# gabegrand/VQA-Counterexamples

Measured on AMD Instinct MI355X. Metric: VQA-CX triplets/sec (24 candidates each), NeuralCX training step, higher is better.
Workload: dtype f32; 1 GPU; configs[1]: NeuralCX MLP train step (fwd+listwise loss/recall+bwd+Adam), synthetic 2048-d feats, 24 candidates, batch 512 per GPU (weak scaling: global batch 512), H=256, L=1, dropout 0.25, fp32; global_batch=512, per_rank_batch=512, candidates=24, dim_h=256, n_layers=1, parallelism=dp1, feature_table_rows=82783

## Files before the change

### vqa-counterexamples_amd/csrc/ncx_api.hip

```cpp
#include "ncx_internal.h"
#include "ncx_dwred.h"
#include "ncx_bf16.h"
#include <stdlib.h>
#include <stdio.h>
#include <atomic>

namespace ncx {

template <int CTRL> __device__ __forceinline__ float dpp_mov(float v) {
    return __builtin_bit_cast(float, __builtin_amdgcn_update_dpp(0, __builtin_bit_cast(int, v), CTRL, 0xF, 0xF, false));
}
__device__ __forceinline__ float lane_bcast(float v, int lane) {
    return __builtin_bit_cast(float, __builtin_amdgcn_readlane(__builtin_bit_cast(int, v), lane));
}
__device__ __forceinline__ float wave_sum(float v) {
    v += dpp_mov<0xB1>(v); v += dpp_mov<0x4E>(v); v += dpp_mov<0x141>(v); v += dpp_mov<0x140>(v);
    return (lane_bcast(v, 0) + lane_bcast(v, 16)) + (lane_bcast(v, 32) + lane_bcast(v, 48));
}
__device__ __forceinline__ float wave_max(float v) {
    v = fmaxf(v, dpp_mov<0xB1>(v)); v = fmaxf(v, dpp_mov<0x4E>(v)); v = fmaxf(v, dpp_mov<0x141>(v)); v = fmaxf(v, dpp_mov<0x140>(v));
    return fmaxf(fmaxf(lane_bcast(v, 0), lane_bcast(v, 16)), fmaxf(lane_bcast(v, 32), lane_bcast(v, 48)));
}

__device__ __forceinline__ u16 f32_to_bf16(float x) { return __builtin_bit_cast(u16, (__bf16)x); }
// ... 542 lines not shown
    if (__syncthreads_or(earlier)) return;
    const int nw = (B + 31) / 32;
    for (int w = threadIdx.x; w < nw; w += 256) bits[w] = 0u;
    __syncthreads();
    for (int j = b + threadIdx.x; j < B; j += 256)
        if (aid[j] == id) atomicOr(&bits[j >> 5], 1u << (j & 31));
    __syncthreads();
    for (int n = threadIdx.x; n < H; n += 256) {
        float s = 0.f;
        for (int w = b >> 5; w < nw; ++w) {
            unsigned m = bits[w];
            while (m) {
                const int j = (w << 5) + __ffs(m) - 1;
                m &= m - 1;
                s += dsh[(long long)j * H + n];
            }
        }
        dggt[(long long)n * A + id] = s;
    }
}

struct EmbPrepArgs {
    const float* dsh; const int* aid; float* dggtT;
    const float* src[3]; float* dst[3]; long long lds_[3]; int cols[3], ldd[3], dcols[3], tile0[4];
    int B, H, A, Hp4;
};
__global__ __launch_bounds__(256) void k_emb_prep(const EmbPrepArgs a, const FixupArgs fix, const Tn8ReduceArgs red) {
    __shared__ unsigned bits[NCX_SCATTER_MAX_B / 32 > 32 * 33 ? NCX_SCATTER_MAX_B / 32 : 32 * 33];
    if ((int)blockIdx.x >= a.B + a.tile0[3]) {
        const int id = blockIdx.x - (a.B + a.tile0[3]);
        const int nfix = fix.valid ? fix.grid_x * 4 : 0;
        if (id < nfix) split_fixup_body<64, 64>(fix, id / 4, id % 4);
        else tn8_reduce_body(red, id - nfix);
        return;
    }
    if ((int)blockIdx.x < a.B) {
        const int b = blockIdx.x, B = a.B;
        const int id = a.aid[b];
        int earlier = 0;
        for (int j = threadIdx.x; j < b; j += 256) earlier |= a.aid[j] == id;
        if (__syncthreads_or(earlier)) return;
        const int nw = (B + 31) / 32;
        for (int w = threadIdx.x; w < nw; w += 256) bits[w] = 0u;
        __syncthreads();
        for (int j = b + threadIdx.x; j < B; j += 256)
            if (a.aid[j] == id) atomicOr(&bits[j >> 5], 1u << (j & 31));
        __syncthreads();
        for (int n = threadIdx.x; n < a.H; n += 256) {
            float s = 0.f;
            for (int w = b >> 5; w < nw; ++w) {
                unsigned m = bits[w];
                while (m) { const int j = (w << 5) + __ffs(m) - 1; m &= m - 1; s += a.dsh[(long long)j * a.H + n]; }
            }
            a.dggtT[(long long)id * a.Hp4 + n] = s;
        }
        return;
    }
    float* tile = (float*)bits;
    int t = blockIdx.x - a.B, e = 0;
    while (e < 2 && t >= a.tile0[e + 1]) ++e;
    t -= a.tile0[e];
    const int tiles_h = (a.dcols[e] + 31) / 32;
    const int th = t % tiles_h, tc = t / tiles_h;
    const int x = threadIdx.x & 31, y = threadIdx.x >> 5;
#pragma unroll
    for (int i = 0; i < 4; ++i) {
        const int h = th * 32 + y + 8 * i, c = tc * 32 + x;
        tile[(y + 8 * i) * 33 + x] = (h < a.H && c < a.cols[e]) ? a.src[e][(long long)h * a.lds_[e] + c] : 0.f;
    }
    __syncthreads();
#pragma unroll
    for (int i = 0; i < 4; ++i) {
        const int c = tc * 32 + y + 8 * i, h = th * 32 + x;
        if (c < a.cols[e] && h < a.dcols[e]) a.dst[e][(long long)c * a.ldd[e] + h] = tile[x * 33 + y + 8 * i];
    }
}

__global__ __launch_bounds__(256) void k_zero_cols(float* __restrict__ p, int rows, long long ld, int cols) {
    const long long i = (long long)blockIdx.x * 256 + threadIdx.x;
    if (i >= (long long)rows * cols) return;
    const int r = (int)(i / cols), c = (int)(i - (long long)r * cols);
    p[(long long)r * ld + c] = 0.f;
}

__global__ __launch_bounds__(256) void k_adam(float* __restrict__ p, const float* __restrict__ g, float* __restrict__ m,
                                              float* __restrict__ v, size_t n, float step_size, float b1, float b2,
                                              float eps, float inv_bc2_sqrt, float gscale) {
    size_t i = ((size_t)blockIdx.x * 256 + threadIdx.x) * 4;
    const size_t stride = (size_t)gridDim.x * 256 * 4;
    for (; i < n; i += stride) {
        if (i + 3 < n) {
            f32x4 pv = *(f32x4*)(p + i), gv = *(const f32x4*)(g + i), mv = *(f32x4*)(m + i), vv = *(f32x4*)(v + i);
#pragma unroll
            for (int j = 0; j < 4; ++j) {
                const float gj = gv[j] * gscale;
                mv[j] = mv[j] + (gj - mv[j]) * (1.f - b1);
                vv[j] = vv[j] * b2 + (1.f - b2) * gj * gj;
                const float den = sqrtf(vv[j]) * inv_bc2_sqrt + eps;
// ... 154 lines not shown
        } else {
            wgs = WgMap{(int)cdiv(u[i].M, bm), (int)cdiv(u[i].N, bn), S}.count();
        }
        u[i].wgs = wgs;
        u[i].slab_elems = S > 1 ? wgs * bm * bn : 0;
    }
    u[U_DW1S].plan.cfg = u[U_DW1C].plan.cfg;
    {
        int bm, bn; cfg_tile(u[U_DW1C].plan.cfg, bm, bn);
        const bool tn8 = dw_tn8_shared_ok(d);
        const long long segs_s[4] = {tn8 ? 0 : d.dv, tn8 ? 0 : d.dq, tn8 ? 0 : d.dz, tn8 ? 0 : d.da};
        const int S = u[U_DW1S].plan.split > 1 ? u[U_DW1S].plan.split : 1;
        u[U_DW1S].tiles = 0; u[U_DW1S].wgs = 0;
        for (int q = 0; q < 4; ++q) {
            if (segs_s[q] == 0) continue;
            u[U_DW1S].tiles += cdiv(H, bm) * cdiv(segs_s[q], bn);
            u[U_DW1S].wgs += WgMap{(int)cdiv(H, bm), (int)cdiv(segs_s[q], bn), S}.count();
        }
        u[U_DW1C].slab_elems = (u[U_DW1C].wgs + u[U_DW1S].wgs) * bm * bn;
        u[U_DW1S].slab_elems = 0;
    }
}

WsLayout ws_layout(const ncx_dims& d) {
    WsLayout w{};
    const size_t M = (size_t)d.B * d.K, H = d.H;
    size_t off = 0;
    auto take = [&](size_t bytes) { size_t o = off; off = align_up(off + bytes, 256); return o; };
    w.idx_k = take(M * 4); w.idx_o = take(M * 4); w.idx_ob = take((size_t)d.B * 4);
    w.mx = take(M * 4); w.inv = take(M * 4);
    w.ldm = pad_to(d.K + 1, 4);
    w.ldgt = (d.flags & NCX_F_BF16) ? d.A : pad_to(d.A, 32);
    w.misc = take(M * w.ldm * 4);
    w.gt = take(H * w.ldgt * 4);
    w.sh = take((size_t)d.B * H * 4);
    for (int l = 0; l < 3; ++l) w.h[l] = l < d.L ? take(M * H * 4) : 0;
    w.dpre[0] = take(M * H * 4);
    w.dpre[1] = d.L >= 2 ? take(M * H * 4) : 0;
    w.dsh = take((size_t)d.B * H * 4);
    w.dgt = take(2 * H * d.A * 4);
    w.dagt = w.dgt + H * d.A * 4;
    w.dgtT = take((size_t)2 * d.A * pad_to(d.H, 4) * 4);
    w.w1aT = take((size_t)2 * d.da * pad_to(d.H, 32) * 4);
    w.dgtT2 = take(dw_tn8_supported(d) ? (size_t)pad_to(d.A, 32) * pad_to(d.H, 4) * 4 : 0);
    w.partial = take((size_t)NCX_PRELUDE_WAVES * H * 4 * 2 + (size_t)NCX_PRELUDE_WAVES * 4 + 256);
    GemmUse u[U_COUNT];
    list_uses(d, u);
    long long slab = 0;
    for (int i = 0; i < U_COUNT; ++i) slab = u[i].slab_elems > slab ? u[i].slab_elems : slab;
    w.slab_bytes = (size_t)slab * 4;
    if (dw_tn8_slab_bytes(d) > w.slab_bytes) w.slab_bytes = dw_tn8_slab_bytes(d);
    w.slab = take(w.slab_bytes);
    {
        long long s2 = u[U_GT].slab_elems;
        if (u[U_SH].slab_elems > s2) s2 = u[U_SH].slab_elems;
        if (u[U_DW1AK].slab_elems > s2) s2 = u[U_DW1AK].slab_elems;
        if (u[U_DE].slab_elems > s2) s2 = u[U_DE].slab_elems;
        w.slab2_bytes = (size_t)s2 * 4;
        w.slab2 = take(w.slab2_bytes);
    }
    w.km_slab = take(dw_km_slab_bytes(d));
    {
        const long long Tm = ks(d.dv) * ((d.flags & NCX_F_V_MULT) ? 2 : 1) + ks(pad_to(d.K + 1, 4)) + ks(d.dz) + ((d.flags & NCX_F_A_EMB) ? ks(d.A) : ks(d.da));
        auto need = [&](long long m, long long n, long long t) { const int sp = main_split(m, n, t); return sp > 1 ? (size_t)sp * m * n * 4 : (size_t)0; };
        size_t b = need((long long)M, (long long)H, Tm);
// ... 390 lines not shown
    if (d.K > 32 || d.H > 256) return NCX_E_DIMS;
    const WsLayout w = ws_layout(d);
    if (workspace_bytes < w.total || ((uintptr_t)workspace & 255)) return NCX_E_WORKSPACE;
    hipStream_t s = (hipStream_t)stream_;
    char* ws = (char*)workspace;
    const int H = d.H;
    const bool aemb = d.flags & NCX_F_A_EMB;
    const bool emb_nt = emb_nt_form(d);
    const int Hp4 = pad_to(H, 4);
    float* dagtT = (float*)(ws + w.dgtT) + (size_t)d.A * Hp4;
    float* dagt = (float*)(ws + w.dagt);
    float* partial = (float*)(ws + w.partial);
    float* part_w = partial;
    float* part_b1 = partial + (size_t)NCX_PRELUDE_WAVES * H;
    float* part_b = partial + (size_t)NCX_PRELUDE_WAVES * H * 2;
    const float dscale = (d.training && d.drop_p > 0.f) ? 1.f / (1.f - d.drop_p) : 1.f;
    const float scale = d.loss_scale > 0.f ? d.loss_scale : 1.f / (float)d.B;
    const int nblk = (int)cdiv(d.B < NCX_PRELUDE_WAVES ? d.B : NCX_PRELUDE_WAVES, 4);
    const bool fuse_l1 = d.L == 1;
    const float* hL = (const float*)(ws + w.h[d.L - 1]);
    float* dpre = (float*)(ws + w.dpre[0]);
    float* dsh = fuse_l1 ? (float*)(ws + w.dsh) : (float*)nullptr;
    float* zb = emb_nt ? dagtT : aemb ? dagt : (float*)nullptr;
    const long long zn = emb_nt ? (long long)d.A * Hp4 : (long long)H * d.A;
#define NCX_TAIL_LAUNCH(KB, FULL) hipLaunchKernelGGL((k_train_tail<KB, FULL>), dim3(nblk * 4), dim3(64), 0, s, hL, p->w_out, p->b_out, gt, d.B, d.K, H, scale, dscale, \
                                               scores, loss_rows, dscores, rank, dpre, dsh, part_w, part_b1, part_b, zb, zn, zchunk)
    const int zchunk = (int)((cdiv(zn, (long long)nblk * 4) + 3) / 4 * 4);
    if (H == 256 && d.K == 24) NCX_TAIL_LAUNCH(24, true);
    else if (d.K <= 8) NCX_TAIL_LAUNCH(8, false); else if (d.K <= 16) NCX_TAIL_LAUNCH(16, false); else if (d.K <= 24) NCX_TAIL_LAUNCH(24, false); else NCX_TAIL_LAUNCH(32, false);
#undef NCX_TAIL_LAUNCH
    NCX_HIP_TRY(hipGetLastError());
    hipLaunchKernelGGL(k_bwd_prelude_finish, dim3((unsigned)cdiv(H, 8), 3), dim3(256), 0, s, (const float*)part_w, (const float*)part_b1,
                       (const float*)part_b, nblk * 4, H, g->w_out, fuse_l1 ? g->b1 : (float*)nullptr, g->b_out,
                       (const float*)loss_rows, (const int*)rank, d.B, loss, hits);
    NCX_HIP_TRY(hipGetLastError());
    return NCX_OK;
}

static int backward_impl(const ncx_dims* dp, const ncx_inputs* in, const ncx_params* p, void* workspace,
                         size_t workspace_bytes, const float* dscores, const ncx_grads* g, void* stream_, int phase);

int ncx_backward(const ncx_dims* dp, const ncx_inputs* in, const ncx_params* p, void* workspace,
                 size_t workspace_bytes, const float* dscores, const ncx_grads* g, void* stream_) {
    return backward_impl(dp, in, p, workspace, workspace_bytes, dscores, g, stream_, 0);
}

int ncx_backward_phase(const ncx_dims* dp, const ncx_inputs* in, const ncx_params* p, void* workspace,
// ... 7 lines not shown
    int rc = check_dims(dp);
    if (rc != NCX_OK) return rc;
    if (!in || !p || !workspace || !g || (!dscores && !(dp->flags & NCX_F_FUSED_TAIL))) return NCX_E_NULL;
    const ncx_dims& d = *dp;
    const bool aemb = d.flags & NCX_F_A_EMB;
    if (!g->answer_embedding || !g->w1 || !g->b1 || !g->w_out || !g->b_out) return NCX_E_NULL;
    if (d.L >= 2 && (!g->w2 || !g->b2)) return NCX_E_NULL;
    if (d.L >= 3 && (!g->w3 || !g->b3)) return NCX_E_NULL;
    const WsLayout w = ws_layout(d);
    if (workspace_bytes < w.total || ((uintptr_t)workspace & 255)) return NCX_E_WORKSPACE;
    hipStream_t s = (hipStream_t)stream_;
    char* ws = (char*)workspace;
    const int M = d.B * d.K, H = d.H;
    const SegOffsets o = seg_offsets(d);
    const long long din = o.din;
    const int* idx_k = (const int*)(ws + w.idx_k); const int* idx_o = (const int*)(ws + w.idx_o);
    const int* idx_ob = (const int*)(ws + w.idx_ob);
    const float* mx = (const float*)(ws + w.mx); const float* inv = (const float*)(ws + w.inv);
    const float* misc = (const float*)(ws + w.misc); const float* gt = (const float*)(ws + w.gt);
    float* dsh = (float*)(ws + w.dsh); float* dgt = (float*)(ws + w.dgt); float* dagt = (float*)(ws + w.dagt);
    const bool emb_nt = emb_nt_form(d);
    const int Hp4 = pad_to(H, 4), Hp32 = pad_to(H, 32);
    float* dgtT = (float*)(ws + w.dgtT); float* dagtT = dgtT + (size_t)d.A * Hp4;
    float* w1akT = (float*)(ws + w.w1aT); float* w1agtT = w1akT + (size_t)d.da * Hp32;
    float* partial = (float*)(ws + w.partial); float* slab = (float*)(ws + w.slab);
    (void)gt;
    GemmUse u[U_COUNT];
    list_uses(d, u);
    const float dscale = (d.training && d.drop_p > 0.f) ? 1.f / (1.f - d.drop_p) : 1.f;
    const int nch = M < NCX_COLSUM_CHUNKS * 8 ? (int)cdiv(M, 8) : NCX_COLSUM_CHUNKS;

    auto colsum = [&](const float* x, const float* wgt, int rows, int cols, float* out) -> int {
        const int ch = rows < NCX_COLSUM_CHUNKS * 8 ? (int)cdiv(rows, 8) : NCX_COLSUM_CHUNKS;
        hipLaunchKernelGGL(k_colsum_partial, dim3((unsigned)cdiv(cols, 256), ch), dim3(256), 0, s, x, wgt, rows, cols, partial);
        hipLaunchKernelGGL(k_colsum_finish, dim3((unsigned)cdiv(cols, 8)), dim3(256), 0, s, (const float*)partial, ch, cols, out);
        return (int)hipGetLastError();
    };
    (void)nch;

    const float* hL = (const float*)(ws + w.h[d.L - 1]);
    float* dpre = (float*)(ws + w.dpre[0]);
    const bool only_de = phase == 4;
    const bool skip_de = phase == 3 || phase == 5;
    const bool do1 = phase != 2 && !only_de, do2 = phase != 1 && phase != 5 && !only_de;
    if (!do1) {
        dpre = (float*)(ws + w.dpre[(d.L - 1) & 1]);
    } else if (d.flags & NCX_F_FUSED_TAIL) {
    } else {
        const int nblk = (int)cdiv(d.B < NCX_PRELUDE_WAVES ? d.B : NCX_PRELUDE_WAVES, 4);
        float* part_w = partial;
        float* part_b1 = partial + (size_t)NCX_PRELUDE_WAVES * H;
        float* part_b = partial + (size_t)NCX_PRELUDE_WAVES * H * 2;
        const bool fuse_l1 = d.L == 1;
        hipLaunchKernelGGL(k_bwd_prelude, dim3(nblk), dim3(256), 0, s, dscores, p->w_out, hL, dpre, fuse_l1 ? dsh : (float*)nullptr,
                           d.B, d.K, H, dscale, part_w, part_b1, part_b,
                           emb_nt ? dagtT : aemb ? dagt : (float*)nullptr, emb_nt ? (long long)d.A * Hp4 : (long long)H * d.A);
        NCX_HIP_TRY(hipGetLastError());
        hipLaunchKernelGGL(k_bwd_prelude_finish, dim3((unsigned)cdiv(H, 8), fuse_l1 ? 2 : 1), dim3(256), 0, s, (const float*)part_w,
                           (const float*)part_b1, (const float*)part_b, nblk * 4, H, g->w_out, fuse_l1 ? g->b1 : (float*)nullptr, g->b_out);
        NCX_HIP_TRY(hipGetLastError());
    }
    int cur = 0;
    for (int l = d.L; l >= 2 && do1; --l) {
        const float* wl = l == 2 ? p->w2 : p->w3;
        float* gw = l == 2 ? g->w2 : g->w3;
        float* gb = l == 2 ? g->b2 : g->b3;
        const float* hprev = (const float*)(ws + w.h[l - 2]);
        rc = colsum(dpre, nullptr, M, H, gb); if (rc) return rc;
        {
            GemmArgs a{}; a.mode = MODE_GROUP; a.nseg = 1; a.M = H;
            a.a[0] = x_plain(dpre, H, M, H); a.b[0] = x_plain(hprev, H, M, H); a.klen[0] = M;
            a.out[0] = gw; a.ldo[0] = H; a.n_cols[0] = H;
            rc = run_gemm(U_DWL, a, FORM_TN, u[U_DWL].plan, slab, w.slab_bytes, nullptr, s); if (rc) return rc;
        }
        {
            float* dnext = (float*)(ws + w.dpre[cur ^ 1]);
            GemmArgs a{}; a.mode = MODE_CHAIN; a.nseg = 1; a.M = M;
            a.a[0] = x_plain(dpre, H, M, H); a.b[0] = x_plain(wl, H, H, H); a.klen[0] = H;
            a.out[0] = dnext; a.ldo[0] = H; a.n_cols[0] = H;
// ... 124 lines not shown
        const Bf16Emb bm = bf16e ? bf16_emb_layout(d, ws + w.bf_emb) : Bf16Emb{};
        if (do2 && bf16e) {
            rc = prof_open(U_DW1AK, se); if (rc) return rc;
            rc = bf16_dw1ak(d, bm, dgt, g->w1, se); if (rc) return rc;
            rc = prof_close(U_DW1AK, se); if (rc) return rc;
        } else if (do2 && tn8_ak) {
            Tn8Prob q{};
            q.A = (const float*)(ws + w.dgtT2); q.rows = pad_to(d.A, 32); q.rows_valid = d.A; q.X = p->answer_embedding; q.ldx = d.da; q.N = d.da;
            q.out = g->w1 + o.a_other; q.ldo = din; q.n_valid = d.da;
            rc = prof_open(U_DW1AK, se); if (rc) return rc;
            rc = dw_tn8_products(d, &q, 1, 0, false, true, nullptr, nullptr, slab, w.slab_bytes, &red_ak, se); if (rc) return rc;
            if (!(do1 && emb_nt)) { rc = dw_reduce_km_tn8(nullptr, true, &red_ak, se); if (rc) return rc; red_ak.n_tiles_total = 0; }
            rc = prof_close(U_DW1AK, se); if (rc) return rc;
        } else if (do2) {
            GemmArgs a{}; a.mode = MODE_CHAIN; a.nseg = 1; a.M = H;
            a.a[0] = x_plain(dgt, d.A, H, d.A); a.b[0] = x_plain(p->answer_embedding, d.da, d.A, d.da); a.klen[0] = d.A;
            a.out[0] = g->w1 + o.a_other; a.ldo[0] = din; a.n_cols[0] = d.da;
            if (do1 && emb_nt && u[U_DW1AK].plan.cfg == CFG_64x64 && !hook_env("NCX_NO_MERGE_FIX")) a.defer_fix = &fix_ak;
            rc = run_gemm(U_DW1AK, a, FORM_NN, u[U_DW1AK].plan, ss ? (float*)(ws + w.slab2) : slab,
                          ss ? w.slab2_bytes : w.slab_bytes, nullptr, se); if (rc) return rc;
        }
        if (do1 && emb_nt) {
            EmbPrepArgs ea{};
            ea.dsh = dsh; ea.aid = in->answer_aids; ea.dggtT = dagtT; ea.B = d.B; ea.H = H; ea.A = d.A; ea.Hp4 = Hp4;
            const float* srcs[3] = {dgt, p->w1 + o.a_other, p->w1 + o.a_gt};
            float* dsts[3] = {dgtT, w1akT, w1agtT};
            const long long ldss[3] = {d.A, din, din};
            const int colss[3] = {tn8_ak ? 0 : d.A, d.da, d.da}, ldds[3] = {Hp4, Hp32, Hp32};
            int tiles = 0;
            for (int e = 0; e < 3; ++e) {
                ea.src[e] = srcs[e]; ea.dst[e] = dsts[e]; ea.lds_[e] = ldss[e]; ea.cols[e] = colss[e]; ea.ldd[e] = ldds[e]; ea.dcols[e] = ldds[e];
                ea.tile0[e] = tiles; tiles += ((ldds[e] + 31) / 32) * ((colss[e] + 31) / 32);
            }
            ea.tile0[3] = tiles;
            hipLaunchKernelGGL(k_emb_prep, dim3(d.B + tiles + (fix_ak.valid ? fix_ak.grid_x * 4 : 0) + red_ak.n_tiles_total * 8), dim3(256), 0, se, ea, fix_ak, red_ak);
            fix_ak.valid = 0; red_ak.n_tiles_total = 0;
            NCX_HIP_TRY(hipGetLastError());
        } else if (do1) {
            hipLaunchKernelGGL(k_scatter_dsh_by_answer, dim3(d.B), dim3(256), 0, se, (const float*)dsh, in->answer_aids, d.B, H, d.A, dagt);
            NCX_HIP_TRY(hipGetLastError());
        }
        if (fix_ak.valid) { rc = run_fixup2(fix_ak, FixupArgs{}, CFG_64x64, se); if (rc) return rc; }
        if (((do1 && !skip_de) || only_de) && bf16e) {
            rc = prof_open(U_DE, se); if (rc) return rc;
            rc = bf16_de(d, bm, dgt, g->answer_embedding, se); if (rc) return rc;
            rc = prof_close(U_DE, se); if (rc) return rc;
        } else if (((do1 && !skip_de) || only_de) && emb_nt) {
            MainArgs a{}; a.M = d.A; a.N = d.da; a.nseg = 2;
            a.seg[0].kind = MK_PLAIN; a.seg[0].a = dgtT;  a.seg[0].lda = Hp4; a.seg[0].klen = Hp4; a.seg[0].b = w1akT;  a.seg[0].ldb = Hp32;
            a.seg[1].kind = MK_PLAIN; a.seg[1].a = dagtT; a.seg[1].lda = Hp4; a.seg[1].klen = Hp4; a.seg[1].b = w1agtT; a.seg[1].ldb = Hp32;
            a.out = g->answer_embedding; a.ldo = d.da;
            a.split = 1;
            rc = prof_open(U_DE, se); if (rc) return rc;
            rc = main_forward(a, se); if (rc) return rc;
            rc = prof_close(U_DE, se); if (rc) return rc;
        } else if ((do1 && !skip_de) || only_de) {
            GemmArgs a{}; a.mode = MODE_CHAIN; a.nseg = 2; a.M = d.A;
            a.a[0] = x_plain(dgt, d.A, H, d.A);  a.b[0] = x_plain(p->w1 + o.a_other, din, H, d.da); a.klen[0] = H;
            a.a[1] = x_plain(dagt, d.A, H, d.A); a.b[1] = x_plain(p->w1 + o.a_gt, din, H, d.da);    a.klen[1] = H;
            a.out[0] = g->answer_embedding; a.ldo[0] = d.da; a.n_cols[0] = d.da;
            rc = run_gemm(U_DE, a, FORM_TN, u[U_DE].plan, ss ? (float*)(ws + w.slab2) : slab, ss ? w.slab2_bytes : w.slab_bytes, nullptr, se); if (rc) return rc;
        }
        if (km_deferred) { rc = run_km(); if (rc) return rc; }
        if (ss) { rc = side_join(ss, s); if (rc) return rc; }
    } else if (do1) {
        NCX_HIP_TRY(hipMemsetAsync(g->answer_embedding, 0, (size_t)d.A * d.da * 4, s));
    }
    return NCX_OK;
}

int ncx_ws_region(const ncx_dims* dp, int32_t which, size_t* offset, size_t* bytes) {
    if (check_dims(dp) != NCX_OK) return NCX_E_DIMS;
    if (!offset || !bytes) return NCX_E_NULL;
    if (which != NCX_WS_DGT && which != NCX_WS_H1 && which != NCX_WS_DPRE1) return NCX_E_FLAGS;
    const WsLayout w = ws_layout(*dp);
    if (which == NCX_WS_H1 || which == NCX_WS_DPRE1) {
// ... 253 lines not shown
```

### vqa-counterexamples_amd/csrc/ncx_dwred.h

```cpp
#pragma once
#include "ncx_internal.h"

namespace ncx {

constexpr int TN8_BM = 256, TN8_BN = 64, TN8_BK = 32, TN8_T = 512;

struct KmReduceArgs { const float* slab; int nz, H, dv; long long din; float* g_vother; float* g_vmult; int nblk; };
template <bool VEC>
__device__ __forceinline__ void km_reduce_body(const KmReduceArgs& r, int blk) {
    constexpr int W = VEC ? 4 : 1;
    typedef float vec __attribute__((ext_vector_type(VEC ? 4 : 1)));
    const long long i = ((long long)blk * 256 + threadIdx.x) * W, n = (long long)r.H * r.dv;
    if (i >= n) return;
    const int h = (int)(i / r.dv), c = (int)(i - (long long)h * r.dv);
    vec vk[DW_KM_SPLIT], vm[DW_KM_SPLIT];
#pragma unroll
    for (int z = 0; z < DW_KM_SPLIT; ++z) {
        const int zz = z < r.nz ? z : r.nz - 1;
        vk[z] = *(const vec*)(r.slab + ((long long)zz * 2 + 0) * n + i);
        vm[z] = *(const vec*)(r.slab + ((long long)zz * 2 + 1) * n + i);
    }
    vec sk = vk[0], sm = vm[0];
#pragma unroll
    for (int z = 1; z < DW_KM_SPLIT; ++z) { const vec zero = {}; sk += z < r.nz ? vk[z] : zero; sm += z < r.nz ? vm[z] : zero; }
// ... 8 lines not shown
    Tn8Prob p[TN8_MAX_PROB];
    int np, n_al, tiles_m, S, al_wgs, R, do_al, do_rest;
    int rest_tiles[TN8_MAX_PROB], rest_steps[TN8_MAX_PROB], rest_tile0[TN8_MAX_PROB], rest_pre[TN8_MAX_PROB + 1];
    int al_tiles, n_tiles_total;
    const float* slab;
};
__device__ __forceinline__ void tn8_reduce_body(const Tn8ReduceArgs& r, int blk) {
    int tile_blk = blk >> 3;
    const int rgp = blk & 7;
    int prob, tile, s_first, s_count, s_stride = 1;
    if (r.do_al && tile_blk < r.al_tiles) {
        prob = 0; tile = tile_blk; s_first = tile * r.S; s_count = r.S;
    } else {
        if (r.do_al) tile_blk -= r.al_tiles;
        prob = r.n_al;
        while (prob + 1 < r.np && tile_blk >= r.rest_tile0[prob + 1]) ++prob;
        tile = tile_blk - r.rest_tile0[prob];
        const long long g0 = (long long)r.rest_pre[prob] + (long long)tile * r.rest_steps[prob], g1 = g0 + r.rest_steps[prob];
        const int w0 = (int)(g0 / r.R), w1 = (int)((g1 - 1) / r.R);
        s_first = r.al_wgs + r.rest_tile0[prob] + tile + w0; s_count = w1 - w0 + 1;
    }
    const Tn8Prob& p = r.p[prob];
    const int tm = tile % r.tiles_m, tn = tile / r.tiles_m;
    __shared__ float tn8_tt[32][TN8_BN + 1];
#pragma unroll
    for (int it = 0; it < 2; ++it) {
        const int f = threadIdx.x + 256 * it, row = rgp * 32 + (f >> 4), c = 4 * (f & 15);
        const float* src = r.slab + (long long)s_first * (TN8_BM * TN8_BN) + row * TN8_BN + c;
        f32x4 sum = {0.f, 0.f, 0.f, 0.f};
        for (int z = 0; z < s_count; z += 8) {
            f32x4 v[8];
#pragma unroll
            for (int j = 0; j < 8; ++j) v[j] = *(const f32x4*)(src + (long long)min(z + j, s_count - 1) * s_stride * (TN8_BM * TN8_BN));
#pragma unroll
            for (int j = 0; j < 8; ++j) sum += z + j < s_count ? v[j] : f32x4{0.f, 0.f, 0.f, 0.f};
        }
        const int h = tm * TN8_BM + row, n = tn * TN8_BN + c;
        float* o = p.out + (long long)h * p.ldo + n;
#pragma unroll
        for (int j = 0; j < 4; ++j) if (n + j < p.n_valid) o[j] = sum[j];
        if (p.outT) {
#pragma unroll
            for (int j = 0; j < 4; ++j) tn8_tt[f >> 4][c + j] = sum[j];
        }
    }
    if (p.outT) {
        __syncthreads();
        const int nl = threadIdx.x >> 2, hq = (threadIdx.x & 3) * 8;
        const int n = tn * TN8_BN + nl, h0 = tm * TN8_BM + rgp * 32 + hq;
        if (n < p.n_valid + p.padT2) {
            float v[8];
#pragma unroll
            for (int j = 0; j < 8; ++j) v[j] = n < p.n_valid ? tn8_tt[hq + j][nl] : 0.f;
#pragma unroll
            for (int j = 0; j < 8; ++j) {
                if (n < p.n_valid) p.outT[(long long)n * p.ldT + h0 + j] = v[j];
                if (p.outT2) p.outT2[(long long)n * p.ldT + h0 + j] = v[j];
            }
        }
    }
}

int dw_tn8_products(const ncx_dims& d, const Tn8Prob* probs, int np, int n_al, bool do_al, bool do_rest, const int* idx_ob, const int* aid,
                    float* slab, size_t slab_bytes, Tn8ReduceArgs* red, hipStream_t s);
int dw_reduce_km_tn8(const KmReduceArgs* km, bool km_vec, const Tn8ReduceArgs* tn, hipStream_t s);
KmReduceArgs dw_km_reduce_args(const ncx_dims& d, const float* slab, float* g_vother, float* g_vmult, long long din, bool* vec);

}
```

### vqa-counterexamples_amd/csrc/ncx_internal.h

```cpp
#pragma once
#include "ncx_common.h"
#include "ncx_gemm.h"

namespace ncx {

enum TileCfg : int { CFG_64x64 = 0, CFG_128x128 = 1, CFG_96x128 = 2, CFG_96x64 = 3, CFG_128x64 = 4 };
enum GemmForm : int { FORM_NT = 0, FORM_TN = 1, FORM_NN = 2 };

int run_gemm_nt(GemmArgs& a, int cfg, hipStream_t s);
int run_fixup2(const FixupArgs& a, const FixupArgs& b, int cfg, hipStream_t s);
int run_gemm_nt_fold(GemmArgs& a, hipStream_t s);
int run_gemm_tn(GemmArgs& a, int cfg, hipStream_t s);
int run_gemm_nn(GemmArgs& a, int cfg, hipStream_t s);
int occupancy_nt(int cfg);
int occupancy_tn(int cfg);
int occupancy_nn(int cfg);

struct SegOffsets {
    int v_orig, v_other, v_mult, v_dist, v_rank, q_emb, z_orig, z_other, a_gt, a_other, din;
};
static inline SegOffsets seg_offsets(const ncx_dims& d) {
    SegOffsets o; int c = 0;
    o.v_orig = c;  c += d.dv;
    o.v_other = c; c += d.dv;
// ... 24 lines not shown
    size_t dsh;
    size_t dgt;
    size_t dagt;
    size_t dgtT;
    size_t dgtT2;
    size_t w1aT;
    size_t partial;
    size_t slab;
    size_t slab_bytes;
    size_t slab2, slab2_bytes;
    size_t xc, wc, dpre_bf, bf_slab;
    size_t bf_emb;
    size_t km_slab;
    size_t mslab, mslab_bytes;
    size_t wpad;
    int ldm;
    int ldgt;
    size_t total;
};
constexpr int NCX_COLSUM_CHUNKS = 256;
constexpr int NCX_PRELUDE_WAVES = 1024;

enum MainKind : int { MK_PLAIN = 0, MK_GATHER = 1, MK_GATHER_MUL = 2, MK_SOFTMAX = 3,
                      MK_VFOLD = 4 };
constexpr int MAIN_MAX_SEG = 5;
struct MainSeg {
    const float* a;
    const int*   idx;
    const int*   idx2;
    const float* lse;
    const float* b;
    const float* b2;
    long long lda, ldb;
    int kind, klen;
};
struct MainArgs {
    MainSeg seg[MAIN_MAX_SEG]; int nseg, M, N, split; float* out; long long ldo; EpiArgs epi;
    float* slab;
    float* dist_out; long long ld_dist;
    unsigned long long* stamps;
    int x6;
};
int main_forward(MainArgs& a, hipStream_t s);
int main_split(long long M, long long N, long long T);
int main_fold_rows_eff(long long M, long long N, int rowdiv);
int main_fold_rows(long long M, long long N);

constexpr int DW_KM_SPLIT = 8;
bool dw_km_supported(const ncx_dims& d);
enum DwKmForm : int { KM_FORM_NONE = 0, KM_FORM_8 = 1, KM_FORM_X6 = 2, KM_FORM_GENERIC = 3, KM_FORM_GROUPED = 4 };
int dw_km_form(const ncx_dims& d);
size_t dw_km_slab_bytes(const ncx_dims& d);
int dw_km(const ncx_dims& d, const float* dpre, const float* feats, const int* idx_k, const int* idx_o, float* slab,
          float* g_vother, float* g_vmult, long long din, hipStream_t s, bool finish = true);
int dw_km_finish(const ncx_dims& d, const float* slab, float* g_vother, float* g_vmult, long long din, const FixupArgs* fix, int fix_cfg,
                 hipStream_t s);
constexpr int TN8_MAX_PROB = 8;
constexpr int TN8_MAX_SEG = 16;
struct Tn8Prob {
    const float* A;
    const float* X; long long ldx;
    const float* lse;
    int gsel;
    int rows, N;
    float* out; long long ldo; int n_valid;
// ... 30 lines not shown
```

### vqa-counterexamples_amd/csrc/ncx_main.h

```cpp
#pragma once
#include "ncx_internal.h"
#include <type_traits>

namespace ncx {

constexpr int MF_BK = 32, MF_P = MF_BK + 4, MF_T = 256;

enum { LK_PLAIN = 0, LK_MUL = 1, LK_SOFTMAX = 2 };
template <int V> struct IntC { static constexpr int value = V; };

constexpr int MF6_P = 80;
template <int BM_, int BN_, int WGM_, int WGN_, int DEPTH_, int OCC_, int T_ = MF_T, bool X6_ = false>
struct MainCfg {
    static constexpr int BM = BM_, BN = BN_, WGM = WGM_, WGN = WGN_, DEPTH = DEPTH_, OCC = OCC_, T = T_;
    static constexpr bool X6 = X6_;
    static constexpr int RP = T / 8;
    static constexpr int BM_LDS = (BM + RP - 1) / RP * RP;
    static constexpr int LDS6 = 2 * 3 * (BM_LDS + BN) * MF6_P;
    static constexpr int LDS_FOLD6 = 2 * (3 * 208 * MF6_P + 8 * 32 * 4 + 128 * MF_P * 4);
    static constexpr int LDS32 = 2 * (BM_LDS + BN) * MF_P * 4;
    static constexpr int LDS = !X6_ ? LDS32 : (LDS_FOLD6 > LDS6 ? (LDS_FOLD6 > LDS32 ? LDS_FOLD6 : LDS32) : (LDS6 > LDS32 ? LDS6 : LDS32));
    static constexpr int LDS_FOLD = BM % 96 == 0 ? 2 * (32 * (T / 64) + 128) * MF_P * 4
                                                 : 2 * (80 + 2 * 64) * MF_P * 4;
};
// ... 100 lines not shown
        const unsigned char* b = lds6 + buf * BUF6 + A6_PL + (wn0 + li) * P6 + 16 * lk;
#pragma unroll
        for (int j = 0; j < (X6 ? WN : 1); ++j)
#pragma unroll
            for (int p = 0; p < 3; ++p) f[j][p] = *(const mbf16x8*)(b + j * 16 * P6 + p * PL6);
    };
    auto mfma6 = [&](const mbf16x8 (&a)[3], const mbf16x8 (&b)[X6 ? WN : 1][3], f32x4 (&c)[WN]) __attribute__((always_inline)) {
        if constexpr (X6) {
#pragma unroll
            for (int j = 0; j < WN; ++j) c[j] = __builtin_amdgcn_mfma_f32_16x16x32_bf16(a[0], b[j][2], c[j], 0, 0, 0);
#pragma unroll
            for (int j = 0; j < WN; ++j) c[j] = __builtin_amdgcn_mfma_f32_16x16x32_bf16(a[1], b[j][1], c[j], 0, 0, 0);
#pragma unroll
            for (int j = 0; j < WN; ++j) c[j] = __builtin_amdgcn_mfma_f32_16x16x32_bf16(a[2], b[j][0], c[j], 0, 0, 0);
#pragma unroll
            for (int j = 0; j < WN; ++j) c[j] = __builtin_amdgcn_mfma_f32_16x16x32_bf16(a[0], b[j][1], c[j], 0, 0, 0);
#pragma unroll
            for (int j = 0; j < WN; ++j) c[j] = __builtin_amdgcn_mfma_f32_16x16x32_bf16(a[1], b[j][0], c[j], 0, 0, 0);
#pragma unroll
            for (int j = 0; j < WN; ++j) c[j] = __builtin_amdgcn_mfma_f32_16x16x32_bf16(a[0], b[j][0], c[j], 0, 0, 0);
        }
    };

    int nsteps[MAIN_MAX_SEG], total_steps = 0;
#pragma unroll
    for (int i = 0; i < MAIN_MAX_SEG; ++i) { nsteps[i] = i < NSEG ? (args.seg[i].klen + BK - 1) / BK : 0; total_steps += nsteps[i]; }
    const int g0 = (int)((long long)total_steps * z / S), g1 = (int)((long long)total_steps * (z + 1) / S);

    f32x4 va[DEPTH][NA], vm[DEPTH][NA], vb[DEPTH][NB];
    typedef unsigned int bu32x4 __attribute__((ext_vector_type(4)));
    __amdgpu_buffer_rsrc_t rsPA = __builtin_amdgcn_make_buffer_rsrc((void*)nullptr, 0, 0, 0x00020000), rsPB = rsPA;
    unsigned roA[NA], roM[NA], roB[NB]; float lse[NA];
    float dacc[NA];
    constexpr int FOLD_DIST_OFF = 2 * (BML + BN) * P > 32 * (MT / 64) * 68 ? 2 * (BML + BN) * P : 32 * (MT / 64) * 68;
#pragma unroll
    for (int i = 0; i < NA; ++i) dacc[i] = 0.f;
    auto setup = [&](auto kind_c, const MainSeg& g) __attribute__((always_inline)) {
        constexpr int KIND = decltype(kind_c)::value;
#pragma unroll
        for (int i = 0; i < NA; ++i) {
            const int r = min(m0 + min(trow + RP * i, BM - 1), M - 1);
            constexpr bool GAT = KIND == MK_GATHER || KIND == MK_GATHER_MUL;
            const unsigned row = GAT ? (unsigned)((giptr)g.idx)[r] : (unsigned)r;
            roA[i] = row * (unsigned)(g.lda * 4);
            roM[i] = KIND == MK_GATHER_MUL ? (unsigned)((giptr)g.idx2)[r] * (unsigned)(g.lda * 4) : roA[i];
            lse[i] = KIND == MK_SOFTMAX ? ((gfptr)g.lse)[r] : 0.f;
        }
#pragma unroll
        for (int i = 0; i < NB; ++i) roB[i] = (unsigned)min(n0 + trow + RP * i, N - 1) * (unsigned)(g.ldb * 4) + 16u * quad;
        rsPA = __builtin_amdgcn_make_buffer_rsrc(const_cast<float*>(g.a), 0, 0xFFFFFFF0u, 0x00020000);
        rsPB = __builtin_amdgcn_make_buffer_rsrc(const_cast<float*>(g.b), 0, 0xFFFFFFF0u, 0x00020000);
    };
    auto issue = [&](auto set_c, auto mul_c, int klen, int nst, int t) __attribute__((always_inline)) {
        constexpr int S = decltype(set_c)::value;
        const int tk4 = min(t, nst - 1) * (BK * 4);
        const unsigned ca4 = (unsigned)min(tk4 + 16 * quad, (klen - 4) * 4);
#pragma unroll
        for (int i = 0; i < NA; ++i) va[S][i] = __builtin_bit_cast(f32x4, (bu32x4)__builtin_amdgcn_raw_buffer_load_b128(rsPA, roA[i] + ca4, 0, 0));
        if (decltype(mul_c)::value) {
#pragma unroll
            for (int i = 0; i < NA; ++i) vm[S][i] = __builtin_bit_cast(f32x4, (bu32x4)__builtin_amdgcn_raw_buffer_load_b128(rsPA, roM[i] + ca4, 0, 0));
        }
#pragma unroll
        for (int i = 0; i < NB; ++i) vb[S][i] = __builtin_bit_cast(f32x4, (bu32x4)__builtin_amdgcn_raw_buffer_load_b128(rsPB, roB[i], tk4, 0));
    };
    typedef IntC<0> S0; typedef IntC<DEPTH - 1> S1;
// ... 760 lines not shown
        add0 = add1; add1 = add2;
        if (use_add) add2 = fetch_add(min(f + 3 * MT, LAST_F));
        if (r >= M || n >= N) continue;
        f32x4 v = *(const f32x4*)(stage + so);
        const int sh = n - nl;
        if (!plain) {
            f32x4 add = addv, msk = {1.f, 1.f, 1.f, 1.f}, gte = {1.f, 1.f, 1.f, 1.f};
            if (e.bias) add += win(e.bias, nl, sh);
            if (e.dropout == 2) msk = win(e.keep_mask + (long long)r * e.ld_mask, nl, sh);
            if (e.gate) gte = win(e.gate + (long long)r * e.ld_gate, nl, sh);
#pragma unroll
            for (int jj = 0; jj < 4; ++jj) {
                float x = v[jj] + add[jj];
                if (e.relu == 1) x = x > 0.f ? x : 0.f;
                else if (e.relu == 2) x = tanhf(x);
                if (e.dropout == 1)
                    x = dropout_keep(e.seed_lo, e.seed_hi, e.layer, (unsigned long long)r * (unsigned)N + (unsigned)(n + jj), e.drop_p) ? x * e.drop_scale : 0.f;
                else if (e.dropout == 2)
                    x = msk[jj] != 0.f ? x * e.drop_scale : 0.f;
                if (e.gate) x = gte[jj] > 0.f ? x * e.gate_scale : 0.f;
                v[jj] = x;
            }
        }
        float* o = dst + (long long)r * ldd + n;
        if (n + 3 < N) *(f32x4u*)o = v;
        else { o[0] = v[0]; if (n + 1 < N) o[1] = v[1]; if (n + 2 < N) o[2] = v[2]; }
    }
    stamp(8);
    if (stamps && tid == 0) stamps[15] = __builtin_amdgcn_s_memrealtime();
}

__global__ __launch_bounds__(256) void k_main_fixup(const MainArgs a) {
    const int M = a.M, N = a.N, S = a.split;
    const int nq = (N + 3) / 4;
    const long long i = (long long)blockIdx.x * 256 + threadIdx.x;
    if (i >= (long long)M * nq) return;
    const int r = (int)(i / nq), n0 = (int)(i - (long long)r * nq) * 4;
    float v[4] = {0.f, 0.f, 0.f, 0.f};
    const long long mn = (long long)M * N, off = (long long)r * N + n0;
    for (int z = 0; z < S; ++z)
#pragma unroll
        for (int j = 0; j < 4; ++j) if (n0 + j < N) v[j] += a.slab[z * mn + off + j];
    const EpiArgs& e = a.epi;
#pragma unroll
    for (int j = 0; j < 4; ++j) {
        const int n = n0 + j;
        if (n >= N) break;
        a.out[(long long)r * a.ldo + n] = apply_epilogue(e, v[j], r, n, N);
    }
}

static inline bool main_fwd_operand_ok(int klen) { return klen >= 4 && klen % 4 == 0; }

template <int K0, int... REST> struct FirstKind { static constexpr int value = K0; };

template <class CFG, bool DIST, int... KINDS>
static inline int launch_main_fwd_seq(MainArgs& a, hipStream_t s) {
    constexpr int lds = FirstKind<KINDS...>::value == MK_VFOLD ? (CFG::LDS_FOLD > CFG::LDS ? CFG::LDS_FOLD : CFG::LDS) : CFG::LDS;
    static DevMask attr{0};
    NCX_HIP_TRY(set_max_lds_once(attr, (const void*)k_main_fwd<CFG, DIST, KINDS...>, lds));
    const int tiles_m = (a.M + CFG::BM - 1) / CFG::BM, tiles_n = (a.N + CFG::BN - 1) / CFG::BN;
    const int S = a.split > 1 ? a.split : 1;
    const int grid = ((tiles_m * S + 7) / 8) * 8 * tiles_n;
    hipLaunchKernelGGL((k_main_fwd<CFG, DIST, KINDS...>), dim3(grid), dim3(CFG::T), lds, s, a);
    NCX_HIP_TRY(hipGetLastError());
    if (S > 1) {
        const long long nthreads = (long long)a.M * ((a.N + 3) / 4);
        hipLaunchKernelGGL(k_main_fixup, dim3((unsigned)((nthreads + 255) / 256)), dim3(256), 0, s, a);
        NCX_HIP_TRY(hipGetLastError());
    }
    return NCX_OK;
}

template <class CFG>
static inline int launch_main_fwd(MainArgs& a, hipStream_t s) {
    if (a.nseg < 1 || a.nseg > MAIN_MAX_SEG || a.M < 1 || a.N < 1) return NCX_E_DIMS;
    for (int i = 0; i < a.nseg; ++i) if (!main_fwd_operand_ok(a.seg[i].klen)) return NCX_E_DIMS;
    if (a.epi.rowadd && a.epi.rowdiv < 3) return NCX_E_DIMS;
    if (a.split > 1 && !a.slab) return NCX_E_WORKSPACE;
    auto is = [&](std::initializer_list<int> ks) { if ((int)ks.size() != a.nseg) return false; int i = 0; for (int k : ks) if (a.seg[i++].kind != k) return false; return true; };
    constexpr int G = MK_GATHER, X = MK_GATHER_MUL, P = MK_PLAIN, S = MK_SOFTMAX;
// ... 21 lines not shown
                    return NCX_E_FLAGS;
                }
            }
            if (is({V, P, P, S})) return launch_main_fwd_seq<CFG, false, V, P, P, S>(a, s);
            if (is({V, P, P, P})) return launch_main_fwd_seq<CFG, false, V, P, P, P>(a, s);
        }
        return NCX_E_FLAGS;
    }
    if constexpr (CFG::X6) return NCX_E_FLAGS;
    else {
    if (a.dist_out) {
        if (a.split > 1 || a.nseg < 3 || a.seg[1].klen % MF_BK) return NCX_E_FLAGS;
        if (is({G, X, P, P, S})) return launch_main_fwd_seq<CFG, true, G, X, P, P, S>(a, s);
        if (is({G, X, P, P, P})) return launch_main_fwd_seq<CFG, true, G, X, P, P, P>(a, s);
        return NCX_E_FLAGS;
    }
    if (is({G, X, P, P, S})) return launch_main_fwd_seq<CFG, false, G, X, P, P, S>(a, s);
    if (is({P}))             return launch_main_fwd_seq<CFG, false, P>(a, s);
    if (is({G}))             return launch_main_fwd_seq<CFG, false, G>(a, s);
    if (is({G, P, P, S}))    return launch_main_fwd_seq<CFG, false, G, P, P, S>(a, s);
    if (is({G, X, P, P, P})) return launch_main_fwd_seq<CFG, false, G, X, P, P, P>(a, s);
    if (is({G, P, P, P}))    return launch_main_fwd_seq<CFG, false, G, P, P, P>(a, s);
    if (is({P, P}))          return launch_main_fwd_seq<CFG, false, P, P>(a, s);
    return NCX_E_FLAGS;
    }
}

}
```

Before: 649,700 triplets/s.

## Skip zero rows of answer-embedding gradient second segment via row permutation mask

Builds a bitmask of answer rows whose aggregated GT gradient is nonzero, filled by the embedding prep kernel and zeroed alongside the gradient buffer. The answer-embedding gradient GEMM gains an MK_PERM mode that compacts rows into set-first order, and tiles holding only unset rows run just the first K segment. This avoids multiplying the mostly-zero second segment when few distinct answers appear in a batch. The same change also pads the tn8 reduce transpose tile in LDS with a slot mapping, likely to avoid bank conflicts. In exchange it adds a prefix-scan and binary search at kernel start and extra LDS.

```diff
diff --git a/vqa-counterexamples_amd/csrc/ncx_api.hip b/vqa-counterexamples_amd/csrc/ncx_api.hip
--- a/vqa-counterexamples_amd/csrc/ncx_api.hip
+++ b/vqa-counterexamples_amd/csrc/ncx_api.hip
@@ -588,6 +588,7 @@
 
 struct EmbPrepArgs {
     const float* dsh; const int* aid; float* dggtT;
+    unsigned* rowmask;
     const float* src[3]; float* dst[3]; long long lds_[3]; int cols[3], ldd[3], dcols[3], tile0[4];
     int B, H, A, Hp4;
 };
@@ -612,6 +613,7 @@
         for (int j = b + threadIdx.x; j < B; j += 256)
             if (a.aid[j] == id) atomicOr(&bits[j >> 5], 1u << (j & 31));
         __syncthreads();
+        int nz = 0;
         for (int n = threadIdx.x; n < a.H; n += 256) {
             float s = 0.f;
             for (int w = b >> 5; w < nw; ++w) {
@@ -619,7 +621,9 @@
                 while (m) { const int j = (w << 5) + __ffs(m) - 1; m &= m - 1; s += a.dsh[(long long)j * a.H + n]; }
             }
             a.dggtT[(long long)id * a.Hp4 + n] = s;
-        }
+            nz |= s != 0.f;
+        }
+        if (__syncthreads_or(nz) && threadIdx.x == 0 && id >= 0 && id < a.A) atomicOr(a.rowmask + (id >> 5), 1u << (id & 31));
         return;
     }
     float* tile = (float*)bits;
@@ -640,6 +644,26 @@
         const int c = tc * 32 + y + 8 * i, h = th * 32 + x;
         if (c < a.cols[e] && h < a.dcols[e]) a.dst[e][(long long)c * a.ldd[e] + h] = tile[x * 33 + y + 8 * i];
     }
+}
+
+__global__ __launch_bounds__(256) void k_de_rowmask(const float* __restrict__ x, int A, int ld, unsigned* __restrict__ mask) {
+    __shared__ unsigned sb[4];
+    const int lane = threadIdx.x & 63, wave = threadIdx.x >> 6;
+    unsigned found = 0u;
+#pragma unroll
+    for (int j = 0; j < 8; ++j) {
+        const int r = blockIdx.x * 32 + wave * 8 + j;
+        bool nz = false;
+        if (r < A)
+            for (int c = 4 * lane; c < ld; c += 256) {
+                const f32x4 v = *(const f32x4*)(x + (long long)r * ld + c);
+                nz |= v[0] != 0.f || v[1] != 0.f || v[2] != 0.f || v[3] != 0.f;
+            }
+        if (__ballot(nz)) found |= 1u << (wave * 8 + j);
+    }
+    if (lane == 0) sb[wave] = found;
+    __syncthreads();
+    if (threadIdx.x == 0) mask[blockIdx.x] = sb[0] | sb[1] | sb[2] | sb[3];
 }
 
 __global__ __launch_bounds__(256) void k_zero_cols(float* __restrict__ p, int rows, long long ld, int cols) {
@@ -840,6 +864,7 @@
     }
 }
 
+static inline int de_mask_words(int A) { return pad_to((A + 31) / 32, 4); }
 WsLayout ws_layout(const ncx_dims& d) {
     WsLayout w{};
     const size_t M = (size_t)d.B * d.K, H = d.H;
@@ -858,7 +883,7 @@
     w.dsh = take((size_t)d.B * H * 4);
     w.dgt = take(2 * H * d.A * 4);
     w.dagt = w.dgt + H * d.A * 4;
-    w.dgtT = take((size_t)2 * d.A * pad_to(d.H, 4) * 4);
+    w.dgtT = take(((size_t)2 * d.A * pad_to(d.H, 4) + de_mask_words(d.A)) * 4);
     w.w1aT = take((size_t)2 * d.da * pad_to(d.H, 32) * 4);
     w.dgtT2 = take(dw_tn8_supported(d) ? (size_t)pad_to(d.A, 32) * pad_to(d.H, 4) * 4 : 0);
     w.partial = take((size_t)NCX_PRELUDE_WAVES * H * 4 * 2 + (size_t)NCX_PRELUDE_WAVES * 4 + 256);
@@ -1295,7 +1320,7 @@
     float* dpre = (float*)(ws + w.dpre[0]);
     float* dsh = fuse_l1 ? (float*)(ws + w.dsh) : (float*)nullptr;
     float* zb = emb_nt ? dagtT : aemb ? dagt : (float*)nullptr;
-    const long long zn = emb_nt ? (long long)d.A * Hp4 : (long long)H * d.A;
+    const long long zn = emb_nt ? (long long)d.A * Hp4 + de_mask_words(d.A) : (long long)H * d.A;
 #define NCX_TAIL_LAUNCH(KB, FULL) hipLaunchKernelGGL((k_train_tail<KB, FULL>), dim3(nblk * 4), dim3(64), 0, s, hL, p->w_out, p->b_out, gt, d.B, d.K, H, scale, dscale, \
                                                scores, loss_rows, dscores, rank, dpre, dsh, part_w, part_b1, part_b, zb, zn, zchunk)
     const int zchunk = (int)((cdiv(zn, (long long)nblk * 4) + 3) / 4 * 4);
@@ -1349,6 +1374,9 @@
     const bool emb_nt = emb_nt_form(d);
     const int Hp4 = pad_to(H, 4), Hp32 = pad_to(H, 32);
     float* dgtT = (float*)(ws + w.dgtT); float* dagtT = dgtT + (size_t)d.A * Hp4;
+    unsigned* de_mask = (unsigned*)(dagtT + (size_t)d.A * Hp4);
+    const char* de_dense_env = getenv("NCX_DE_DENSE");
+    const bool de_sparse = emb_nt && d.A <= MAIN_PERM_MAX_ROWS && !(de_dense_env && atoi(de_dense_env));
     float* w1akT = (float*)(ws + w.w1aT); float* w1agtT = w1akT + (size_t)d.da * Hp32;
     float* partial = (float*)(ws + w.partial); float* slab = (float*)(ws + w.slab);
     (void)gt;
@@ -1381,7 +1409,7 @@
         const bool fuse_l1 = d.L == 1;
         hipLaunchKernelGGL(k_bwd_prelude, dim3(nblk), dim3(256), 0, s, dscores, p->w_out, hL, dpre, fuse_l1 ? dsh : (float*)nullptr,
                            d.B, d.K, H, dscale, part_w, part_b1, part_b,
-                           emb_nt ? dagtT : aemb ? dagt : (float*)nullptr, emb_nt ? (long long)d.A * Hp4 : (long long)H * d.A);
+                           emb_nt ? dagtT : aemb ? dagt : (float*)nullptr, emb_nt ? (long long)d.A * Hp4 + de_mask_words(d.A) : (long long)H * d.A);
         NCX_HIP_TRY(hipGetLastError());
         hipLaunchKernelGGL(k_bwd_prelude_finish, dim3((unsigned)cdiv(H, 8), fuse_l1 ? 2 : 1), dim3(256), 0, s, (const float*)part_w,
                            (const float*)part_b1, (const float*)part_b, nblk * 4, H, g->w_out, fuse_l1 ? g->b1 : (float*)nullptr, g->b_out);
@@ -1552,7 +1580,7 @@
         }
         if (do1 && emb_nt) {
             EmbPrepArgs ea{};
-            ea.dsh = dsh; ea.aid = in->answer_aids; ea.dggtT = dagtT; ea.B = d.B; ea.H = H; ea.A = d.A; ea.Hp4 = Hp4;
+            ea.dsh = dsh; ea.aid = in->answer_aids; ea.dggtT = dagtT; ea.rowmask = de_mask; ea.B = d.B; ea.H = H; ea.A = d.A; ea.Hp4 = Hp4;
             const float* srcs[3] = {dgt, p->w1 + o.a_other, p->w1 + o.a_gt};
             float* dsts[3] = {dgtT, w1akT, w1agtT};
             const long long ldss[3] = {d.A, din, din};
@@ -1577,11 +1605,17 @@
             rc = prof_close(U_DE, se); if (rc) return rc;
         } else if (((do1 && !skip_de) || only_de) && emb_nt) {
             MainArgs a{}; a.M = d.A; a.N = d.da; a.nseg = 2;
-            a.seg[0].kind = MK_PLAIN; a.seg[0].a = dgtT;  a.seg[0].lda = Hp4; a.seg[0].klen = Hp4; a.seg[0].b = w1akT;  a.seg[0].ldb = Hp32;
-            a.seg[1].kind = MK_PLAIN; a.seg[1].a = dagtT; a.seg[1].lda = Hp4; a.seg[1].klen = Hp4; a.seg[1].b = w1agtT; a.seg[1].ldb = Hp32;
+            const int kind = de_sparse ? MK_PERM : MK_PLAIN;
+            a.seg[0].kind = kind; a.seg[0].a = dgtT;  a.seg[0].lda = Hp4; a.seg[0].klen = Hp4; a.seg[0].b = w1akT;  a.seg[0].ldb = Hp32;
+            a.seg[1].kind = kind; a.seg[1].a = dagtT; a.seg[1].lda = Hp4; a.seg[1].klen = Hp4; a.seg[1].b = w1agtT; a.seg[1].ldb = Hp32;
             a.out = g->answer_embedding; a.ldo = d.da;
             a.split = 1;
+            a.rowmask = de_sparse ? de_mask : nullptr;
             rc = prof_open(U_DE, se); if (rc) return rc;
+            if (de_sparse && only_de) {
+                hipLaunchKernelGGL(k_de_rowmask, dim3((unsigned)cdiv(d.A, 32)), dim3(256), 0, se, (const float*)dagtT, d.A, Hp4, de_mask);
+                NCX_HIP_TRY(hipGetLastError());
+            }
             rc = main_forward(a, se); if (rc) return rc;
             rc = prof_close(U_DE, se); if (rc) return rc;
         } else if ((do1 && !skip_de) || only_de) {
diff --git a/vqa-counterexamples_amd/csrc/ncx_dwred.h b/vqa-counterexamples_amd/csrc/ncx_dwred.h
--- a/vqa-counterexamples_amd/csrc/ncx_dwred.h
+++ b/vqa-counterexamples_amd/csrc/ncx_dwred.h
@@ -54,7 +54,8 @@
     }
     const Tn8Prob& p = r.p[prob];
     const int tm = tile % r.tiles_m, tn = tile / r.tiles_m;
-    __shared__ float tn8_tt[32][TN8_BN + 1];
+    __shared__ float tn8_tt[56][TN8_BN + 1];
+    auto slot = [](int h) { return ((h >> 3) << 4) + (h & 7); };
 #pragma unroll
     for (int it = 0; it < 2; ++it) {
         const int f = threadIdx.x + 256 * it, row = rgp * 32 + (f >> 4), c = 4 * (f & 15);
@@ -73,7 +74,7 @@
         for (int j = 0; j < 4; ++j) if (n + j < p.n_valid) o[j] = sum[j];
         if (p.outT) {
 #pragma unroll
-            for (int j = 0; j < 4; ++j) tn8_tt[f >> 4][c + j] = sum[j];
+            for (int j = 0; j < 4; ++j) tn8_tt[slot(f >> 4)][c + j] = sum[j];
         }
     }
     if (p.outT) {
@@ -83,7 +84,7 @@
         if (n < p.n_valid + p.padT2) {
             float v[8];
 #pragma unroll
-            for (int j = 0; j < 8; ++j) v[j] = n < p.n_valid ? tn8_tt[hq + j][nl] : 0.f;
+            for (int j = 0; j < 8; ++j) v[j] = n < p.n_valid ? tn8_tt[slot(hq + j)][nl] : 0.f;
 #pragma unroll
             for (int j = 0; j < 8; ++j) {
                 if (n < p.n_valid) p.outT[(long long)n * p.ldT + h0 + j] = v[j];
diff --git a/vqa-counterexamples_amd/csrc/ncx_internal.h b/vqa-counterexamples_amd/csrc/ncx_internal.h
--- a/vqa-counterexamples_amd/csrc/ncx_internal.h
+++ b/vqa-counterexamples_amd/csrc/ncx_internal.h
@@ -70,7 +70,8 @@
 constexpr int NCX_PRELUDE_WAVES = 1024;
 
 enum MainKind : int { MK_PLAIN = 0, MK_GATHER = 1, MK_GATHER_MUL = 2, MK_SOFTMAX = 3,
-                      MK_VFOLD = 4 };
+                      MK_VFOLD = 4,
+                      MK_PERM = 5 };
 constexpr int MAIN_MAX_SEG = 5;
 struct MainSeg {
     const float* a;
@@ -88,7 +89,9 @@
     float* dist_out; long long ld_dist;
     unsigned long long* stamps;
     int x6;
+    const unsigned* rowmask;
 };
+constexpr int MAIN_PERM_MAX_ROWS = 8192;
 int main_forward(MainArgs& a, hipStream_t s);
 int main_split(long long M, long long N, long long T);
 int main_fold_rows_eff(long long M, long long N, int rowdiv);
diff --git a/vqa-counterexamples_amd/csrc/ncx_main.h b/vqa-counterexamples_amd/csrc/ncx_main.h
--- a/vqa-counterexamples_amd/csrc/ncx_main.h
+++ b/vqa-counterexamples_amd/csrc/ncx_main.h
@@ -146,10 +146,46 @@
         }
     };
 
+    constexpr bool PERM = K0 == MK_PERM;
+    static_assert(!PERM || (NSEG == 2 && K1 == MK_PERM && MT == 256 && BM <= 256 && !X6 && !DIST), "MK_PERM: the two-segment sequence on the 4-wave forms");
+    int* const s_prow = (int*)(mf_smem + CFG::LDS / 4);
+    int perm_set = 0;
+    if constexpr (PERM) {
+        unsigned* const s_w = (unsigned*)(s_prow + BM);
+        int* const s_pre = (int*)(s_w + 256);
+        int* const s_tot = s_pre + 256;
+        const int nw = (M + 31) >> 5;
+        const unsigned wv = tid < nw ? ((const __attribute__((address_space(1))) unsigned*)args.rowmask)[tid] : 0u;
+        const int cnt = __popc(wv);
+        int inc = cnt;
+#pragma unroll
+        for (int o = 1; o < 64; o <<= 1) { const int v = __shfl_up(inc, o, 64); inc += lane >= o ? v : 0; }
+        if (lane == 63) s_tot[wave] = inc;
+        s_w[tid] = wv;
+        __syncthreads();
+        int wbase = 0;
+#pragma unroll
+        for (int q = 0; q < 4; ++q) { const int tq = s_tot[q]; wbase += q < wave ? tq : 0; perm_set += tq; }
+        s_pre[tid] = wbase + inc - cnt;
+        __syncthreads();
+        if (tid < BM) {
+            const int p = min(m0 + tid, M - 1);
+            const bool set = p < perm_set;
+            const int q = set ? p : p - perm_set;
+            auto before = [&](int t) { return set ? s_pre[t] : 32 * t - s_pre[t]; };
+            int lo = 0, hi = nw - 1;
+            while (lo < hi) { const int mid = (lo + hi + 1) >> 1; if (before(mid) <= q) lo = mid; else hi = mid - 1; }
+            unsigned x = set ? s_w[lo] : ~s_w[lo];
+            for (int k = q - before(lo); k > 0; --k) x &= x - 1;
+            s_prow[tid] = min(max(32 * lo + __ffs(x) - 1, 0), M - 1);
+        }
+        __syncthreads();
+    }
     int nsteps[MAIN_MAX_SEG], total_steps = 0;
 #pragma unroll
     for (int i = 0; i < MAIN_MAX_SEG; ++i) { nsteps[i] = i < NSEG ? (args.seg[i].klen + BK - 1) / BK : 0; total_steps += nsteps[i]; }
-    const int g0 = (int)((long long)total_steps * z / S), g1 = (int)((long long)total_steps * (z + 1) / S);
+    const int g0 = (int)((long long)total_steps * z / S);
+    const int g1 = PERM && m0 >= perm_set ? nsteps[0] : (int)((long long)total_steps * (z + 1) / S);
 
     f32x4 va[DEPTH][NA], vm[DEPTH][NA], vb[DEPTH][NB];
     typedef unsigned int bu32x4 __attribute__((ext_vector_type(4)));
@@ -165,7 +201,7 @@
         for (int i = 0; i < NA; ++i) {
             const int r = min(m0 + min(trow + RP * i, BM - 1), M - 1);
             constexpr bool GAT = KIND == MK_GATHER || KIND == MK_GATHER_MUL;
-            const unsigned row = GAT ? (unsigned)((giptr)g.idx)[r] : (unsigned)r;
+            const unsigned row = GAT ? (unsigned)((giptr)g.idx)[r] : KIND == MK_PERM ? (unsigned)s_prow[r - m0] : (unsigned)r;
             roA[i] = row * (unsigned)(g.lda * 4);
             roM[i] = KIND == MK_GATHER_MUL ? (unsigned)((giptr)g.idx2)[r] * (unsigned)(g.lda * 4) : roA[i];
             lse[i] = KIND == MK_SOFTMAX ? ((gfptr)g.lse)[r] : 0.f;
@@ -972,7 +1008,7 @@
                 v[jj] = x;
             }
         }
-        float* o = dst + (long long)r * ldd + n;
+        float* o = dst + (long long)(PERM ? s_prow[f / QR] : r) * ldd + n;
         if (n + 3 < N) *(f32x4u*)o = v;
         else { o[0] = v[0]; if (n + 1 < N) o[1] = v[1]; if (n + 2 < N) o[2] = v[2]; }
     }
@@ -1006,7 +1042,8 @@
 
 template <class CFG, bool DIST, int... KINDS>
 static inline int launch_main_fwd_seq(MainArgs& a, hipStream_t s) {
-    constexpr int lds = FirstKind<KINDS...>::value == MK_VFOLD ? (CFG::LDS_FOLD > CFG::LDS ? CFG::LDS_FOLD : CFG::LDS) : CFG::LDS;
+    constexpr int lds = (FirstKind<KINDS...>::value == MK_VFOLD ? (CFG::LDS_FOLD > CFG::LDS ? CFG::LDS_FOLD : CFG::LDS) : CFG::LDS) +
+                        (FirstKind<KINDS...>::value == MK_PERM ? (CFG::BM + 256 + 256 + 8) * 4 : 0);
     static DevMask attr{0};
     NCX_HIP_TRY(set_max_lds_once(attr, (const void*)k_main_fwd<CFG, DIST, KINDS...>, lds));
     const int tiles_m = (a.M + CFG::BM - 1) / CFG::BM, tiles_n = (a.N + CFG::BN - 1) / CFG::BN;
@@ -1074,6 +1111,11 @@
     if (is({G, X, P, P, P})) return launch_main_fwd_seq<CFG, false, G, X, P, P, P>(a, s);
     if (is({G, P, P, P}))    return launch_main_fwd_seq<CFG, false, G, P, P, P>(a, s);
     if (is({P, P}))          return launch_main_fwd_seq<CFG, false, P, P>(a, s);
+    if (is({MK_PERM, MK_PERM})) {
+        const EpiArgs& e = a.epi;
+        if (!a.rowmask || a.split > 1 || a.M > MAIN_PERM_MAX_ROWS || e.rowadd || e.bias || e.relu || e.dropout || e.gate) return NCX_E_FLAGS;
+        if constexpr (CFG::BM <= 96) return launch_main_fwd_seq<CFG, false, MK_PERM, MK_PERM>(a, s);
+    }
     return NCX_E_FLAGS;
     }
 }
```

Result: no change. 655,600 triplets/s, median of 6 (+0.9%).
